# emtiyaz/vmp-for-svae

Hardware: AMD Instinct MI355X
Metric: vmp_step_datapoints_per_sec (higher is better)
Workload: dtype f32

## Files before the change

### vmp-for-svae_amd/csrc/vmp_mix.hip

```cpp
#include "vmp_common.h"
#include "vmp_linalg.h"
#include <stdlib.h>
#include <type_traits>

using namespace vmp;

namespace {

constexpr int TR = 64;
constexpr int LS = 68;
constexpr int MAX_NW = 8;
constexpr int MAX_NW1 = 8;
constexpr int max_nw(int KT) { return KT == 1 ? MAX_NW1 : MAX_NW; }
constexpr int MAX_BLOCKS = 1024;

struct PassArgs {
    const float* x;
    const float* r_in;
    const float* u_in;
    const uint8_t* mask;
    const float* pivot;
    const float* pack;
    float* r_out;
    float* u_out;
// ... 472 lines not shown
            } else {
                group(integral_constant<bool, false>{}, integral_constant<int, 0>{});
                group(integral_constant<bool, false>{}, integral_constant<int, 1>{});
                group(integral_constant<bool, false>{}, integral_constant<int, 2>{});
                group(integral_constant<bool, false>{}, integral_constant<int, 3>{});
            }

            if constexpr (STATS) {
                bf16x8 b[FT][3];
#pragma unroll
                for (int ft = 0; ft < FT; ++ft)
#pragma unroll
                    for (int t = 0; t < 3; ++t)
                        b[ft][t] = __builtin_bit_cast(bf16x8, u32x4{Bs[ft][t][0], Bs[ft][t][1], Bs[ft][t][2], Bs[ft][t][3]});
#pragma unroll
                for (int kt = 0; kt < KT; ++kt) {
                    bf16x8 av[3], rv[3];
#pragma unroll
                    for (int t = 0; t < 3; ++t) {
                        av[t] = __builtin_bit_cast(bf16x8, u32x4{As[kt][t][0], As[kt][t][1], As[kt][t][2], As[kt][t][3]});
                        if constexpr (SMM) rv[t] = __builtin_bit_cast(bf16x8, u32x4{Rs[kt][t][0], Rs[kt][t][1], Rs[kt][t][2], Rs[kt][t][3]});
                    }
#pragma unroll
                    for (int ta = 0; ta < MOM_TERMS; ++ta) {
#pragma unroll
                        for (int tb = 0; tb + ta < MOM_TERMS; ++tb) {
#pragma unroll
                            for (int ft = 0; ft < FT; ++ft) {
                                if (ta + tb == 0) acc[kt][ft] = __builtin_amdgcn_mfma_f32_16x16x32_bf16(av[ta], b[ft][tb], acc[kt][ft], 0, 0, 0);
                                else acs[kt][ft] = __builtin_amdgcn_mfma_f32_16x16x32_bf16(av[ta], b[ft][tb], acs[kt][ft], 0, 0, 0);
                            }
                        }
                        if constexpr (SMM) {
                            if (ta == 0) nacc[kt] = __builtin_amdgcn_mfma_f32_16x16x32_bf16(rv[ta], b[0][0], nacc[kt], 0, 0, 0);
                            else nacs[kt] = __builtin_amdgcn_mfma_f32_16x16x32_bf16(rv[ta], b[0][0], nacs[kt], 0, 0, 0);
                        }
                    }
                }
            }
        }

        if constexpr (STATS) {
            if (((row0 - lo) / TR) % VMP_MOM_FLUSH == VMP_MOM_FLUSH - 1 || row0 + TR >= hi) {
#pragma unroll
                for (int kt = 0; kt < KT; ++kt) {
#pragma unroll
                    for (int c = 0; c < 4; ++c) {
                        if constexpr (SMM) dn[kt][c] += (double)nacc[kt][c] + (double)nacs[kt][c];
#pragma unroll
                        for (int ft = 0; ft < FT; ++ft) dacc[kt][ft][c] += (double)acc[kt][ft][c] + (double)acs[kt][ft][c];
                    }
                    nacc[kt] = f32x4{0.f, 0.f, 0.f, 0.f};
                    nacs[kt] = f32x4{0.f, 0.f, 0.f, 0.f};
#pragma unroll
                    for (int ft = 0; ft < FT; ++ft) { acc[kt][ft] = f32x4{0.f, 0.f, 0.f, 0.f}; acs[kt][ft] = f32x4{0.f, 0.f, 0.f, 0.f}; }
                }
            }
        }
        __builtin_amdgcn_wave_barrier();
    }

    PASS_TS(2);
    if constexpr (STATS) pass_epilogue<D, KT, FLAV>(a, smem, dacc, dn, lane, wave, nw);
}


constexpr int AIS = 36;

struct FinArgs {
    const double* partials;
    const double* stats_in;
    int nblk, K, flavour, src, do_post;
    const float *alpha0, *beta0, *m0, *C0, *v0, *kappa;
    const float* pivot;
    float *alpha, *beta, *m, *C, *v, *xbar, *S, *pi, *pack;
    double* pack64;
    double* stats_out;
    double* peer[VMP_EXCH_MAX_RANKS];
    int nranks, rank;
    unsigned long long iter;
    int* status;
#ifdef VMP_DEBUG_TS
    long long* dbg_t;
#endif
};

#ifdef VMP_DEBUG_TS
#define FIN_TS(i) do { if (a.dbg_t && blockIdx.x == 0 && tid == 0) { a.dbg_t[i] = clock64(); if ((i) == 0) a.dbg_t[6] = wall_clock64(); if ((i) == 5) a.dbg_t[7] = wall_clock64(); } } while (0)
#else
#define FIN_TS(i) do { } while (0)
#endif
#ifdef VMP_DEBUG_TS
#define FIN_TSX(i, t) do { if (a.dbg_t && blockIdx.x == 0 && tid == (t)) a.dbg_t[i] = clock64(); } while (0)
#else
#define FIN_TSX(i, t) do { } while (0)
#endif

template <int D>
__device__ void finalize_block(const FinArgs& a, const int k, const int tid, const int nthreads);

template <int D> constexpr int xdl_wave_floats() { return Geo<D>::XROWS * LS + TR * AIS; }

template <int D, int FLAV, bool STATS, int MT = 3, bool GEN = true>
__device__ __forceinline__ void pass_xdl_body(const PassArgs& a) {
    using G = Geo<D>;
    constexpr int FT = G::FT, KT = 1;
    constexpr bool SMM = (FLAV == VMP_SMM);
    constexpr int DP = (D + 1) / 2;
    extern __shared__ __attribute__((aligned(16))) float smem[];
    const int lane = threadIdx.x & 63, wave = threadIdx.x >> 6, nw = blockDim.x >> 6;
    const int K = GEN ? a.K : 16;
    PASS_TS(0);
    float* xl = smem + wave * xdl_wave_floats<D>();
    unsigned* ai = reinterpret_cast<unsigned*>(xl + G::XROWS * LS);
    constexpr int ONE = D, ZERO = D + 1;
    const int ppos = (lane & ~15) + 4 * (lane & 3) + ((lane >> 2) & 3);

    const bool vec = a.vec_ok != 0;
    long long lo, hi;
    if (a.rpw_b == a.rpw) {
        lo = ((long long)blockIdx.x * nw + wave) * a.rpw;
        hi = lo + a.rpw;
    } else {
        const int hw = nw >> 1;
        const long long base = (long long)blockIdx.x * hw * (a.rpw + a.rpw_b);
        lo = wave < hw ? base + wave * a.rpw : base + hw * a.rpw + (wave - hw) * a.rpw_b;
        hi = lo + (wave < hw ? a.rpw : a.rpw_b);
    }
    if (hi > a.N) hi = a.N;
    float xr[D];
    {
        const long long n = lo + lane;
#pragma unroll
        for (int j = 0; j < D; ++j) xr[j] = 0.f;
        if (n < hi) load_row<D>(a.x + n * D, xr, vec);
    }
    const int i16 = lane & 15, kk = lane >> 4;
    float pv[D];
    {
        const float* __restrict__ pp = a.pivot ? a.pivot : a.x;
        const bool hasp = a.pivot != nullptr;
#pragma unroll
        for (int j = 0; j < D; ++j) { const float v = pp[j]; pv[j] = hasp ? v : 0.f; }
#pragma unroll
        for (int j = 0; j < D; ++j) pv[j] = __builtin_bit_cast(float, __builtin_amdgcn_readfirstlane(__builtin_bit_cast(int, pv[j])));
    }

    constexpr int NS = D < 4 ? D : 4;
    constexpr int NB = D > 4 ? D - 4 : 0;
    constexpr int QK = 3 * NS + 4 * NB, QS = QK | 1;
    static_assert(16 * QS * 4 <= xdl_wave_floats<D>(), "the operand image must fit the LDS of a one-wave launch");
    u32x4 Bsm[NS], B1[NB > 0 ? NB : 1], B2[NB > 0 ? NB : 1];
    v2f pch;
    float pua, pub;
    {
        const bool on = i16 < K;
        const float* __restrict__ pc = a.pack + (on ? i16 : 0) * G::PACK + D + G::TRI;
        const float c0 = pc[0], c1 = pc[1], c2 = pc[2], c3 = pc[3];
        pch.x = on ? c0 : -INFINITY;
        pch.y = on ? c1 : 0.f;
        pua = on ? c2 : 0.f;
        pub = on ? c3 : 1.f;
    }
    {
        u32x4* img = reinterpret_cast<u32x4*>(smem);
        for (int it = threadIdx.x; it < 16 * D; it += blockDim.x) {
            const int k = it / D, i = it - k * D;
            const bool on = k < K;
            const float* __restrict__ p = a.pack + (on ? k : 0) * G::PACK;
            const int tri = i * (i + 1) / 2;
            float mr[D], wr[D];
#pragma unroll
            for (int j = 0; j < D; ++j) { mr[j] = p[j]; wr[j] = p[D + tri + j]; }
            double bi = 0.0;
#pragma unroll
            for (int j = 0; j < D; ++j)
                if (j <= i) bi -= (double)wr[j] * ((double)mr[j] - (double)pv[j]);
            unsigned tb[3];
            split_bf16<3>(v2f{(float)bi, 0.f}, tb);
            const unsigned bias0 = (tb[0] & 0xffffu) | (tb[1] << 16), bias1 = tb[2] & 0xffffu;
            unsigned th[4] = {0u, 0u, 0u, 0u}, tm[4] = {0u, 0u, 0u, 0u}, tl[4] = {0u, 0u, 0u, 0u};
#pragma unroll
            for (int q = 0; q < DP; ++q) {
                const int j0 = 2 * q, j1 = 2 * q + 1;
                const float wa = j0 <= i ? wr[j0] : 0.f;
                const float wb = (j1 <= i && j1 < D) ? wr[j1 < D ? j1 : 0] : 0.f;
                unsigned t3[3];
                split_bf16<3>(v2f{wa, wb}, t3);
                th[q] = t3[0]; tm[q] = t3[1]; tl[q] = t3[2];
            }
            const u32x4 zero = u32x4{0u, 0u, 0u, 0u};
            const u32x4 bias = on ? u32x4{bias0, bias1, 0u, 0u} : zero;
            if (i < NS) {
                u32x4* o = img + k * QS + 3 * i;
                o[0] = on ? u32x4{th[0], th[1], tm[0], tm[1]} : zero;
                o[1] = on ? u32x4{th[0], th[1], tl[0], tl[1]} : zero;
                o[2] = bias;
            } else {
                u32x4* o = img + k * QS + 3 * NS + 4 * (i - 4);
                o[0] = on ? u32x4{th[0], th[1], th[2], th[3]} : zero;
                o[1] = on ? u32x4{tm[0], tm[1], tm[2], tm[3]} : zero;
                o[2] = on ? u32x4{tl[0], tl[1], tl[2], tl[3]} : zero;
                o[3] = bias;
            }
        }
        __syncthreads();
        const u32x4* q = img + i16 * QS;
        const int s0 = kk == 1 ? 1 : (kk == 3 ? 2 : 0);
#pragma unroll
        for (int i = 0; i < NS; ++i) Bsm[i] = q[3 * i + s0];
        if constexpr (NB > 0) {
            const int s1 = kk == 1 ? 3 : (kk == 2 ? 1 : 0), s2 = kk == 0 ? 2 : (kk == 1 ? 0 : 1);
#pragma unroll
            for (int ib = 0; ib < NB; ++ib) {
                B1[ib] = q[3 * NS + 4 * ib + s1];
                const u32x4 w2 = q[3 * NS + 4 * ib + s2];
                B2[ib] = kk == 3 ? u32x4{0u, 0u, 0u, 0u} : w2;
            }
        }
        __syncthreads();
    }
    xl[ONE * LS + lane] = 1.0f;
    xl[ZERO * LS + lane] = 0.0f;
    {
        u32x4 ones = u32x4{0x3F803F80u, 0x00003F80u, 0u, 0u}, zeros = u32x4{0u, 0u, 0u, 0u};
        *reinterpret_cast<u32x4*>(ai + lane * AIS + 12) = ones;
        *reinterpret_cast<u32x4*>(ai + lane * AIS + 16) = zeros;
    }
    const int rho = 4 * (i16 & 3) + (i16 >> 2);
    const int offA1 = rho * AIS + (kk == 1 ? 12 : (kk == 3 ? 4 : 0));
    const int offA2 = rho * AIS + (kk == 0 ? 0 : (kk == 1 ? 8 : (kk == 2 ? 4 : 16)));
    const int offA3 = rho * AIS + (kk == 3 ? 12 : 20 + 4 * kk);

    int offA[FT], offB[FT];
#pragma unroll
    for (int ft = 0; ft < FT; ++ft) {
        const int f = ft * 16 + i16;
        int ra = ZERO, rb = ZERO;
        if (f == 0) { ra = ONE; rb = ONE; }
        else if (f <= D) { ra = f - 1; rb = ONE; }
        else if (f < G::F) {
            int p = f - D - 1, d = 0;
            while (p >= D - d) { p -= D - d; ++d; }
            ra = d; rb = d + p;
        }
        offA[ft] = ra * LS + 4 * kk;
        offB[ft] = rb * LS + 4 * kk;
    }

    f32x4 acc[KT][FT], acs[KT][FT];
    double dacc[KT][FT][4];
    double dn[KT][4];
    float nsum = 0.f;
    double dnl = 0.0;
#pragma unroll
    for (int c = 0; c < 4; ++c) dn[0][c] = 0.0;
#pragma unroll
    for (int ft = 0; ft < FT; ++ft) {
        acc[0][ft] = f32x4{0.f, 0.f, 0.f, 0.f};
        acs[0][ft] = f32x4{0.f, 0.f, 0.f, 0.f};
#pragma unroll
        for (int c = 0; c < 4; ++c) dacc[0][ft][c] = 0.0;
    }

#ifdef VMP_DEBUG_TS
    asm volatile("" :: "v"(xr[0]), "v"(pv[0]), "v"(pch.x), "v"(Bsm[0][0]));
    asm volatile("s_waitcnt vmcnt(0)" ::: "memory");
#endif
    PASS_TS(1);
    long long row0 = lo, tbase = 0;
    int trows = TR;
    auto stage = [&](auto whole_c) __attribute__((always_inline)) {
        constexpr bool WHOLE = decltype(whole_c)::value;
        {
            const bool valid = WHOLE || row0 + lane < hi;
            float xs[2 * DP];
#pragma unroll
            for (int j = 0; j < 2 * DP; ++j) xs[j] = (valid && j < D) ? xr[j < D ? j : 0] - pv[j < D ? j : 0] : 0.f;
#pragma unroll
            for (int j = 0; j < D; ++j) xl[j * LS + ppos] = xs[j];
            unsigned th[4] = {0u, 0u, 0u, 0u}, tm[4] = {0u, 0u, 0u, 0u}, tl[4] = {0u, 0u, 0u, 0u};
#pragma unroll
            for (int q = 0; q < DP; ++q) {
                unsigned t3[3];
                split_bf16<3>(v2f{xs[2 * q], xs[2 * q + 1]}, t3);
                th[q] = t3[0]; tm[q] = t3[1]; tl[q] = t3[2];
            }
            *reinterpret_cast<u32x4*>(ai + lane * AIS) = u32x4{th[0], th[1], th[2], th[3]};
            *reinterpret_cast<u32x4*>(ai + lane * AIS + 4) = u32x4{tm[0], tm[1], tm[2], tm[3]};
            *reinterpret_cast<u32x4*>(ai + lane * AIS + 8) = u32x4{tl[0], tl[1], tl[2], tl[3]};
            *reinterpret_cast<u32x4*>(ai + lane * AIS + 20) = u32x4{th[0], th[1], th[0], th[1]};
            *reinterpret_cast<u32x4*>(ai + lane * AIS + 24) = u32x4{tm[0], tm[1], th[0], th[1]};
            *reinterpret_cast<u32x4*>(ai + lane * AIS + 28) = u32x4{tl[0], tl[1], tm[0], tm[1]};
            long long nb = row0 + TR;
            if (!GEN && WHOLE && nb < hi && nb > hi - TR) nb = hi - TR;
            const long long n2 = nb + lane;
#pragma unroll
            for (int j = 0; j < D; ++j) xr[j] = 0.f;
            if (n2 < hi) load_row<D>(a.x + n2 * D, xr, vec);
        }
        __builtin_amdgcn_wave_barrier();
        tbase = (row0 + kk) * (WHOLE ? 16 : K) + i16;
    };
    int othr = 0;
    auto body = [&](auto full_c, auto n0_v, auto ovl_c) __attribute__((always_inline)) {
        constexpr bool FULL = decltype(full_c)::value;
        constexpr bool LINE = !std::is_same<decltype(n0_v), int>::value;
        constexpr bool OVL = decltype(ovl_c)::value;
        static_assert(!OVL || LINE, "only a straight-line tile overlaps");
        const int n0 = n0_v;
        unsigned As[3][4], Bs[FT][3][4];
        auto subtile = [&](auto jj_c) __attribute__((always_inline)) {
            constexpr int jj = decltype(jj_c)::value;
            const int n16 = n0 + 16 * jj;
            if (!FULL && n16 >= trows) {
                if constexpr (STATS) {
#pragma unroll
                    for (int t = 0; t < 3; ++t) {
                        As[t][2 * jj] = 0u; As[t][2 * jj + 1] = 0u;
#pragma unroll
                        for (int ft = 0; ft < FT; ++ft) { Bs[ft][t][2 * jj] = 0u; Bs[ft][t][2 * jj + 1] = 0u; }
                    }
                }
                return;
            }
            f32x4 y[D];
            {
                const bf16x8 a3 = __builtin_bit_cast(bf16x8, *reinterpret_cast<const u32x4*>(ai + n16 * AIS + offA3));
#pragma unroll
                for (int i = 0; i < NS; ++i)
                    y[i] = __builtin_amdgcn_mfma_f32_16x16x32_bf16(a3, __builtin_bit_cast(bf16x8, Bsm[i]), f32x4{0.f, 0.f, 0.f, 0.f}, 0, 0, 0);
            }
            if constexpr (NB > 0) {
                const bf16x8 a1 = __builtin_bit_cast(bf16x8, *reinterpret_cast<const u32x4*>(ai + n16 * AIS + offA1));
                const bf16x8 a2 = __builtin_bit_cast(bf16x8, *reinterpret_cast<const u32x4*>(ai + n16 * AIS + offA2));
#pragma unroll
                for (int i = 0; i < NB; ++i)
                    y[4 + i] = __builtin_amdgcn_mfma_f32_16x16x32_bf16(a1, __builtin_bit_cast(bf16x8, B1[i]), f32x4{0.f, 0.f, 0.f, 0.f}, 0, 0, 0);
#pragma unroll
                for (int i = 0; i < NB; ++i)
                    y[4 + i] = __builtin_amdgcn_mfma_f32_16x16x32_bf16(a2, __builtin_bit_cast(bf16x8, B2[i]), y[4 + i], 0, 0, 0);
            }
            f32x4 q4 = y[0] * y[0], q4b = f32x4{0.f, 0.f, 0.f, 0.f};
#pragma unroll
            for (int i = 1; i < D; ++i) {
                if (i & 1) q4b = __builtin_elementwise_fma(y[i], y[i], q4b);
                else q4 = __builtin_elementwise_fma(y[i], y[i], q4);
            }
            q4 += q4b;
            v2f lg[2], uu[2], rr[2], w[2];
#pragma unroll
            for (int h = 0; h < 2; ++h) {
                const v2f qh = v2f{q4[2 * h], q4[2 * h + 1]};
                lg[h] = pk_const_minus_scaled(qh, pch);
                if constexpr (SMM) uu[h] = v2f{pua * __builtin_amdgcn_rcpf(qh.x + pub), pua * __builtin_amdgcn_rcpf(qh.y + pub)};
            }
            if constexpr (LINE) {
                static_assert(FULL, "straight-line tiles are whole tiles");
                const float mxs = row16_rs4_max(lg[0], lg[1]);
                lg[0] = v2f{__builtin_amdgcn_exp2f(lg[0].x - row16_bcast_bank<0>(mxs)), __builtin_amdgcn_exp2f(lg[0].y - row16_bcast_bank<1>(mxs))};
                lg[1] = v2f{__builtin_amdgcn_exp2f(lg[1].x - row16_bcast_bank<2>(mxs)), __builtin_amdgcn_exp2f(lg[1].y - row16_bcast_bank<3>(mxs))};
                const float invs = __builtin_amdgcn_rcpf(row16_rs4_sum(lg[0], lg[1]));
                rr[0] = v2f{lg[0].x * row16_bcast_bank<0>(invs), lg[0].y * row16_bcast_bank<1>(invs)};
                rr[1] = v2f{lg[1].x * row16_bcast_bank<2>(invs), lg[1].y * row16_bcast_bank<3>(invs)};
#pragma unroll
                for (int h = 0; h < 2; ++h) w[h] = SMM ? rr[h] * uu[h] : rr[h];
            } else {
                v2f mx[2], ssum[2];
#pragma unroll
                for (int h = 0; h < 2; ++h) {
                    mx[h] = row16_max2(lg[h]);
                    lg[h] = v2f{__builtin_amdgcn_exp2f(lg[h].x - mx[h].x), __builtin_amdgcn_exp2f(lg[h].y - mx[h].y)};
                    ssum[h] = row16_sum2(lg[h]);
                }
#pragma unroll
                for (int h = 0; h < 2; ++h) {
                    v2f inv = v2f{__builtin_amdgcn_rcpf(ssum[h].x), __builtin_amdgcn_rcpf(ssum[h].y)};
                    if constexpr (!FULL) {
                        const bool va = row0 + n16 + 8 * h + kk < hi, vb = row0 + n16 + 8 * h + 4 + kk < hi;
                        inv = v2f{va ? inv.x : 0.f, vb ? inv.y : 0.f};
                    }
                    rr[h] = lg[h] * inv;
                    w[h] = SMM ? rr[h] * uu[h] : rr[h];
                }
            }
#pragma unroll
            for (int v = 0; v < 4; ++v) {
                const float rv = rr[v >> 1][v & 1];
                if constexpr (FULL) {
                    float* __restrict__ ro = a.r_out + tbase + (long long)(n16 + 4 * v) * 16;
                    __builtin_nontemporal_store(rv, ro);
                    if constexpr (SMM) __builtin_nontemporal_store(uu[v >> 1][v & 1], a.u_out + tbase + (long long)(n16 + 4 * v) * 16);
                    if constexpr (!LINE)
                        if (a.logr_out) a.logr_out[tbase + (long long)(n16 + 4 * v) * 16] = logf(rv);
                } else {
                    const bool sv = (row0 + n16 + 4 * v + kk < hi) && i16 < K;
                    const long long o = tbase + (long long)(n16 + 4 * v) * K;
                    if (sv) {
                        a.r_out[o] = rv;
                        if constexpr (SMM) a.u_out[o] = uu[v >> 1][v & 1];
                        if (a.logr_out) a.logr_out[o] = logf(rv);
                    }
                }
            }
            if constexpr (LINE) {
                if (a.logr_out) {
#pragma unroll
                    for (int v = 0; v < 4; ++v) a.logr_out[tbase + (long long)(n16 + 4 * v) * 16] = logf(rr[v >> 1][v & 1]);
                }
            }
            if constexpr (STATS) {
                if constexpr (OVL) {
#pragma unroll
                    for (int h = 0; h < 2; ++h) {
                        const bool ka = n16 + 8 * h >= othr, kb = n16 + 8 * h + 4 >= othr;
                        w[h] = v2f{ka ? w[h].x : 0.f, kb ? w[h].y : 0.f};
                        if constexpr (SMM) rr[h] = v2f{ka ? rr[h].x : 0.f, kb ? rr[h].y : 0.f};
                    }
                }
                unsigned t3[3];
#pragma unroll
                for (int h = 0; h < 2; ++h) {
                    split_bf16<MT>(w[h], t3);
#pragma unroll
                    for (int t = 0; t < 3; ++t) As[t][2 * jj + h] = t3[t];
                }
                if constexpr (SMM) nsum += (rr[0].x + rr[0].y) + (rr[1].x + rr[1].y);
#pragma unroll
                for (int ft = 0; ft < FT; ++ft) {
                    const f32x4 fa = *reinterpret_cast<const f32x4*>(&xl[offA[ft] + n16]);
                    const f32x4 fb = *reinterpret_cast<const f32x4*>(&xl[offB[ft] + n16]);
                    const f32x4 pr = fa * fb;
#pragma unroll
                    for (int h = 0; h < 2; ++h) {
                        split_bf16<MT>(v2f{pr[2 * h], pr[2 * h + 1]}, t3);
#pragma unroll
                        for (int t = 0; t < 3; ++t) Bs[ft][t][2 * jj + h] = t3[t];
                    }
                }
            }
        };
        using std::integral_constant;
        subtile(integral_constant<int, 0>{});
        subtile(integral_constant<int, 1>{});

        if constexpr (STATS) {
            bf16x8 b[FT][3];
#pragma unroll
            for (int ft = 0; ft < FT; ++ft)
#pragma unroll
                for (int t = 0; t < 3; ++t)
                    b[ft][t] = __builtin_bit_cast(bf16x8, u32x4{Bs[ft][t][0], Bs[ft][t][1], Bs[ft][t][2], Bs[ft][t][3]});
            bf16x8 av[3];
#pragma unroll
            for (int t = 0; t < 3; ++t) av[t] = __builtin_bit_cast(bf16x8, u32x4{As[t][0], As[t][1], As[t][2], As[t][3]});
#pragma unroll
            for (int ta = 0; ta < MT; ++ta) {
#pragma unroll
                for (int tb = 0; tb + ta < MT; ++tb) {
#pragma unroll
                    for (int ft = 0; ft < FT; ++ft) {
                        if (ta + tb == 0) acc[0][ft] = __builtin_amdgcn_mfma_f32_16x16x32_bf16(av[ta], b[ft][tb], acc[0][ft], 0, 0, 0);
                        else acs[0][ft] = __builtin_amdgcn_mfma_f32_16x16x32_bf16(av[ta], b[ft][tb], acs[0][ft], 0, 0, 0);
                    }
                }
            }
        }
    };

    auto flush = [&]() __attribute__((always_inline)) {
        if constexpr (STATS) {
            if (((row0 - lo) / TR) % VMP_MOM_FLUSH == VMP_MOM_FLUSH - 1 || row0 + TR >= hi) {
#pragma unroll
                for (int c = 0; c < 4; ++c) {
#pragma unroll
                    for (int ft = 0; ft < FT; ++ft) dacc[0][ft][c] += (double)acc[0][ft][c] + (double)acs[0][ft][c];
                }
                if constexpr (SMM) { dnl += (double)nsum; nsum = 0.f; }
#pragma unroll
                for (int ft = 0; ft < FT; ++ft) { acc[0][ft] = f32x4{0.f, 0.f, 0.f, 0.f}; acs[0][ft] = f32x4{0.f, 0.f, 0.f, 0.f}; }
            }
        }
        __builtin_amdgcn_wave_barrier();
    };

    using std::integral_constant;
    using T_ = integral_constant<bool, true>;
    using F_ = integral_constant<bool, false>;
    if constexpr (!GEN) {
        for (; row0 + TR <= hi; row0 += TR) {
            stage(T_{});
            body(T_{}, integral_constant<int, 0>{}, F_{});
            body(T_{}, integral_constant<int, 32>{}, F_{});
            flush();
        }
        PASS_TS(6);
        if (row0 < hi && hi - lo >= TR) {
            const int done = TR - (int)(hi - row0);
            row0 = hi - TR;
            othr = done - kk;
            stage(T_{});
            if (done < 32) body(T_{}, integral_constant<int, 0>{}, T_{});
            body(T_{}, integral_constant<int, 32>{}, T_{});
            flush();
        }
    } else {
        if (K == 16) {
            for (; row0 + TR <= hi; row0 += TR) {
                stage(T_{});
                body(T_{}, integral_constant<int, 0>{}, F_{});
                body(T_{}, integral_constant<int, 32>{}, F_{});
                flush();
            }
        }
        PASS_TS(6);
        for (; row0 < hi; row0 += TR) {
            trows = (hi - row0 < TR) ? (int)(hi - row0) : TR;
            stage(F_{});
#pragma unroll 1
            for (int n0 = 0; n0 < trows; n0 += 32) {
                const bool full = (K == 16) && (n0 + 32 <= trows);
                if (full) body(T_{}, n0, F_{});
                else body(F_{}, n0, F_{});
            }
            flush();
        }
    }

    PASS_TS(2);
    if constexpr (STATS && SMM) {
        double tot = dnl;
        {
            int lo = __double2loint(tot), hi = __double2hiint(tot);
            tot += __hiloint2double(__shfl_xor(hi, 32), __shfl_xor(lo, 32));
            lo = __double2loint(tot); hi = __double2hiint(tot);
            tot += __hiloint2double(__shfl_xor(hi, 16), __shfl_xor(lo, 16));
        }
#pragma unroll
        for (int c = 0; c < 4; ++c) {
            const int src = 4 * kk + c;
            const int lo = __shfl(__double2loint(tot), src), hi = __shfl(__double2hiint(tot), src);
            dn[0][c] = __hiloint2double(hi, lo);
        }
    }
    if constexpr (STATS) pass_epilogue<D, 1, FLAV>(a, smem, dacc, dn, lane, wave, nw);
}

template <int D, int FLAV, bool STATS, int MT = 3>
__global__ __launch_bounds__(MAX_NW1 * WAVE) void pass_xdl_kernel(PassArgs a) {
    pass_xdl_body<D, FLAV, STATS, MT, true>(a);
}
template <int D, int FLAV, bool STATS, int MT = 3>
__global__ __launch_bounds__(MAX_NW1 * WAVE) void pass_xdl_overlap_kernel(PassArgs a) {
    pass_xdl_body<D, FLAV, STATS, MT, false>(a);
}

template <int D>
__device__ void write_pack(float* pack, int k, const double* m, const double* W ,
                           double c, double h, double ua, double ub) {
    using G = Geo<D>;
    float* p = pack + k * G::PACK;
    int idx = D;
    for (int j = 0; j < D; ++j) p[j] = (float)m[j];
    for (int i = 0; i < D; ++i)
        for (int j = 0; j <= i; ++j) p[idx++] = (float)W[i * D + j];
    const double LOG2E = 1.4426950408889634074;
    p[idx++] = (float)(c * LOG2E); p[idx++] = (float)(h * LOG2E); p[idx++] = (float)ua; p[idx++] = (float)ub;
}

__device__ __forceinline__ double fast_rsqrt_d(double x) {
    double y = __builtin_amdgcn_rsq(x);
    y = y * (1.5 - 0.5 * x * y * y);
    y = y * (1.5 - 0.5 * x * y * y);
    return y;
}

template <int D>
__device__ __forceinline__ void wave_chol_inverse(const double* A, int lane, double (&X)[D], double& sumlog, bool& ok) {
    double row[D], rd[D];
#pragma unroll
    for (int e = 0; e < D; ++e)
        row[e] = lane < D ? 0.5 * (A[lane * D + e] + A[e * D + lane]) : (e == lane ? 1.0 : 0.0);
    ok = true;
    double mydiag = 1.0;
#pragma unroll
    for (int j = 0; j < D; ++j) {
        double t = row[j];
#pragma unroll
        for (int p = 0; p < j; ++p) t -= row[p] * readlane_d(row[p], j);
        const double sj = readlane_d(t, j);
        ok = ok && (sj > 0.0);
        rd[j] = fast_rsqrt_d(sj);
        if (lane == j) mydiag = sj;
        row[j] = lane >= j ? t * rd[j] : 0.0;
    }
    double lg = lane < D ? 0.5 * log(mydiag) : 0.0;
    sumlog = 0.0;
#pragma unroll
    for (int j = 0; j < D; ++j) sumlog += readlane_d(lg, j);
#pragma unroll
    for (int i = 0; i < D; ++i) {
        double acc = (i == lane) ? 1.0 : 0.0;
#pragma unroll
        for (int p = 0; p < i; ++p) acc -= readlane_d(row[p], i) * X[p];
        X[i] = acc * rd[i];
    }
}

template <int D>
__device__ void estep_constants(int k, int flavour, double alpha_k, double alpha_sum, double beta_k, double v_k,
                                double logdetP, double kap, double& c, double& h, double& ua, double& ub, double& elp) {
    const double LOG2 = 0.69314718055994530942, PI = 3.14159265358979323846;
    elp = digamma_d(alpha_k) - digamma_d(alpha_sum);
    double sdg = 0.0;
    if (flavour == VMP_GMM) {
        for (int i = 0; i < D; ++i) sdg += digamma_d(0.5 * (v_k + 1.0 + i));
        const double ld = (logdetP > log(1e-20)) ? logdetP : 0.0;
        const double eld = sdg + D * LOG2 + ld;
        c = elp + 0.5 * eld - 0.5 * (D / beta_k);
        h = 0.5; ua = 1.0; ub = 1.0;
    } else {
        for (int i = 0; i < D; ++i) sdg += digamma_d(0.5 * (v_k + i));
        const double eld = sdg + D * LOG2 + logdetP;
        h = 0.5 * (D + kap);
        c = lgamma(0.5 * (D + kap)) - lgamma(0.5 * kap) - 0.5 * D * log(kap * PI) + elp + 0.5 * eld
            - h * (D / beta_k) + log(kap);
        ua = D + kap;
        ub = D / beta_k + kap;
    }
}

constexpr int FIN_THREADS = 1024;
constexpr int FIN_MAX_GROUPS = FIN_THREADS / 64;

__device__ __forceinline__ void st_pack(const FinArgs& a, int idx, double v) {
    a.pack[idx] = (float)v;
    if (a.pack64) a.pack64[idx] = v;
}

template <int D>
__device__ void finalize_block(const FinArgs& a, const int k, const int tid, const int nthreads) {
    using G = Geo<D>;
    __shared__ double part[FIN_MAX_GROUPS][64];
    __shared__ double st[G::SW];
    __shared__ double ntot;
    __shared__ double Ck[D * D], mk[D], sp[8], scal[8];
    __shared__ double alpha0s[VMP_MAX_K];
    const int K = a.K;
    const int FIN_GROUPS = nthreads >> 6;
    const bool post = a.do_post != 0;
    const bool smm = a.flavour == VMP_SMM;
    const double beta0 = post ? (double)a.beta0[k] : 0.0, v0 = post ? (double)a.v0[k] : 0.0;
    const double alpha0 = post ? (double)a.alpha0[k] : 0.0;
    const double kap = (post && smm) ? (double)a.kappa[k] : 0.0;
    bool shifted = (a.src == 0) && (a.pivot != nullptr);
    double m0d = 0.0, m0e = 0.0, C0de = 0.0, cd = 0.0, ce = 0.0;
    if (tid < D * D) {
        const int d = tid / D, e = tid % D;
        if (post) { m0d = a.m0[k * D + d]; m0e = a.m0[k * D + e]; C0de = a.C0[(k * D + d) * D + e]; }
        if (shifted) { cd = a.pivot[d]; ce = a.pivot[e]; }
    }
    if (post && tid < K) alpha0s[tid] = a.alpha0[tid];

    FIN_TS(0);
    if (a.src == 0) {
        constexpr int PX = G::PF + 1;
        const int f = tid & 63, g = tid >> 6;
        const double* __restrict__ mine = a.partials + (long long)k * MAX_BLOCKS * PX;
        int lo = 0, hi = f - (1 + D);
#pragma unroll
        for (int j = 0; j < D; ++j)
            if (lo == j && hi >= D - j) { hi -= D - j; lo = j + 1; }
        hi += lo;
        for (int lg = g; lg < FIN_MAX_GROUPS; lg += FIN_GROUPS) {
            double s = 0.0;
            for (int b0 = lg; b0 < a.nblk; b0 += FIN_MAX_GROUPS * 16) {
                double v1[16];
                const int fc = f < PX ? f : PX - 1;
#pragma unroll
                for (int i = 0; i < 16; ++i) {
                    const int b = b0 + i * FIN_MAX_GROUPS;
                    const int bc = b < a.nblk ? b : a.nblk - 1;
                    v1[i] = mine[(long long)bc * PX + fc];
                }
#pragma unroll
                for (int i = 0; i < 16; ++i) {
                    const bool in = b0 + i * FIN_MAX_GROUPS < a.nblk;
                    v1[i] = (in && f < PX) ? v1[i] : 0.0;
                }
#pragma unroll
                for (int i = 0; i < 16; ++i) s += v1[i];
            }
            part[lg][f] = s;
        }
        __syncthreads();
        FIN_TS(1);
        if (tid < 64) {
            double t1 = 0.0;
            for (int gg = 0; gg < FIN_MAX_GROUPS; ++gg) t1 += part[gg][tid];
            if (f == G::F) st[0] = t1;
            if (f == 0) st[1] = t1;
            if (f == G::PF) ntot = t1;
            if (f >= 1 && f < 1 + D) st[2 + (f - 1)] = t1;
            if (f >= 1 + D && f < G::F) { st[2 + D + lo * D + hi] = t1; st[2 + D + hi * D + lo] = t1; }
        }
    } else {
        for (int i = tid; i < G::SW; i += nthreads) st[i] = a.stats_in[(long long)k * G::SW + i];
        if (tid == 0) {
            double t = 0.0;
            for (int j = 0; j < K; ++j) t += a.stats_in[(long long)j * G::SW];
            ntot = t;
        }
    }
    __syncthreads();
    if (a.nranks >= 1) {
        constexpr int SWP = (G::SW + 1 + 7) & ~7;
        const int par = (int)(a.iter & 1), G_ = a.nranks;
        double val = 0.0;
        if (tid < G::SW) {
            val = st[tid];
            if (shifted && tid >= 2) {
                const double W = st[1];
                if (tid < 2 + D) {
                    val += W * (double)a.pivot[tid - 2];
                } else {
                    const int d = (tid - 2 - D) / D, e = (tid - 2 - D) % D;
                    const double pd = a.pivot[d], pe = a.pivot[e];
                    val += pd * st[2 + e] + st[2 + d] * pe + W * pd * pe;
                }
            }
        } else if (tid == G::SW) {
            val = ntot;
        }
        if (tid <= G::SW) {
            for (int g = 0; g < G_; ++g) {
                double* slot = a.peer[g] + (((size_t)par * G_ + a.rank) * K + k) * SWP;
                __hip_atomic_store(slot + tid, val, __ATOMIC_RELAXED, __HIP_MEMORY_SCOPE_SYSTEM);
            }
            __builtin_amdgcn_fence(__ATOMIC_RELEASE, "");
            asm volatile("s_waitcnt vmcnt(0)" ::: "memory");
        }
        __syncthreads();
        if (tid == 0) {
            __builtin_amdgcn_fence(__ATOMIC_RELEASE, "");
            asm volatile("s_waitcnt vmcnt(0)" ::: "memory");
            for (int g = 0; g < G_; ++g) {
                unsigned long long* fl = reinterpret_cast<unsigned long long*>(a.peer[g] + (size_t)2 * G_ * K * SWP);
                __hip_atomic_store(fl + ((size_t)par * G_ + a.rank) * K + k, a.iter + 1ull, __ATOMIC_RELAXED, __HIP_MEMORY_SCOPE_SYSTEM);
            }
        }
        double* mine = a.peer[a.rank];
        if (tid < G_) {
            const unsigned long long* fl = reinterpret_cast<const unsigned long long*>(mine + (size_t)2 * G_ * K * SWP)
                                           + ((size_t)par * G_ + tid) * K + k;
            const long long t0 = wall_clock64();
            bool ok = false;
            while (!ok) {
                ok = __hip_atomic_load(fl, __ATOMIC_RELAXED, __HIP_MEMORY_SCOPE_SYSTEM) == a.iter + 1ull;
                if (!ok) {
                    if (wall_clock64() - t0 > 400000000ll) break;
                    __builtin_amdgcn_s_sleep(8);
                }
            }
            if (!ok && a.status) *a.status = 1;
        }
        __syncthreads();
        if (tid == 0) __builtin_amdgcn_fence(__ATOMIC_ACQUIRE, "");
        __syncthreads();
        if (tid <= G::SW) {
            double s2 = 0.0;
            for (int g = 0; g < G_; ++g)
                s2 += __hip_atomic_load(mine + (((size_t)par * G_ + g) * K + k) * SWP + tid, __ATOMIC_RELAXED, __HIP_MEMORY_SCOPE_SYSTEM);
            if (tid < G::SW) st[tid] = s2; else ntot = s2;
        }
        shifted = false;
        cd = 0.0; ce = 0.0;
        __syncthreads();
    }
    if (a.stats_out) {
        for (int i = tid; i < G::SW; i += nthreads) {
            double val = st[i];
            if (shifted && i >= 2) {
                const double W = st[1];
                if (i < 2 + D) {
                    val += W * (double)a.pivot[i - 2];
                } else {
                    const int d = (i - 2 - D) / D, e = (i - 2 - D) % D;
                    const double pd = a.pivot[d], pe = a.pivot[e];
                    val += pd * st[2 + e] + st[2 + d] * pe + W * pd * pe;
                }
            }
            a.stats_out[(long long)k * G::SW + i] = val;
        }
    }
    if (!a.do_post) return;

    const double Nk = st[0], Wk = smm ? st[1] : st[0];
    const double* sx = st + 2;
    const double* sxx = st + 2 + D;
    const double den = smm ? (Wk + 1e-20) : Wk;
    const bool empty = (!smm) && !(Wk != 0.0);
    const double alpha_k = alpha0 + Nk;
    const double beta_k = beta0 + Wk;
    const double v_k = smm ? (v0 + Nk) : (v0 + Nk + 1.0);
    FIN_TS(2);
    if (tid < D * D) {
        const int d = tid / D, e = tid % D;
// ... 749 lines not shown
```

Measured before the change: 24.41 billion.

## Interleave MFMA energy computation with softmax post-processing across 16-row subtiles

Adds a specialised path for non-generic D=8, MT=2 stats passes that software-pipelines each 64-row tile. The MFMA energy products for the next 16-row subtile are issued while the softmax, stores and bf16 splitting of the current subtile run, with sched_barriers pinning the order. The aim is to hide MFMA latency behind VALU and transcendental work. It duplicates the body logic in a new code path, which raises register pressure and adds maintenance risk.

```diff
diff --git a/vmp-for-svae_amd/csrc/vmp_mix.hip b/vmp-for-svae_amd/csrc/vmp_mix.hip
--- a/vmp-for-svae_amd/csrc/vmp_mix.hip
+++ b/vmp-for-svae_amd/csrc/vmp_mix.hip
@@ -798,6 +798,7 @@
         __builtin_amdgcn_wave_barrier();
         tbase = (row0 + kk) * (WHOLE ? 16 : K) + i16;
     };
+    constexpr bool IL = !GEN && STATS && D == 8 && MT == 2;
     int othr = 0;
     auto body = [&](auto full_c, auto n0_v, auto ovl_c) __attribute__((always_inline)) {
         constexpr bool FULL = decltype(full_c)::value;
@@ -984,21 +985,189 @@
     using T_ = integral_constant<bool, true>;
     using F_ = integral_constant<bool, false>;
     if constexpr (!GEN) {
-        for (; row0 + TR <= hi; row0 += TR) {
-            stage(T_{});
-            body(T_{}, integral_constant<int, 0>{}, F_{});
-            body(T_{}, integral_constant<int, 32>{}, F_{});
-            flush();
-        }
-        PASS_TS(6);
-        if (row0 < hi && hi - lo >= TR) {
-            const int done = TR - (int)(hi - row0);
-            row0 = hi - TR;
-            othr = done - kk;
-            stage(T_{});
-            if (done < 32) body(T_{}, integral_constant<int, 0>{}, T_{});
-            body(T_{}, integral_constant<int, 32>{}, T_{});
-            flush();
+        if constexpr (IL) {
+            auto epart_a = [&](const int n16, f32x4 (&y)[D]) __attribute__((always_inline)) {
+                const bf16x8 a3 = __builtin_bit_cast(bf16x8, *reinterpret_cast<const u32x4*>(ai + n16 * AIS + offA3));
+#pragma unroll
+                for (int i = 0; i < NS; ++i)
+                    y[i] = __builtin_amdgcn_mfma_f32_16x16x32_bf16(a3, __builtin_bit_cast(bf16x8, Bsm[i]), f32x4{0.f, 0.f, 0.f, 0.f}, 0, 0, 0);
+            };
+            auto epart_b = [&](const int n16, f32x4 (&y)[D]) __attribute__((always_inline)) {
+                const bf16x8 a1 = __builtin_bit_cast(bf16x8, *reinterpret_cast<const u32x4*>(ai + n16 * AIS + offA1));
+                const bf16x8 a2 = __builtin_bit_cast(bf16x8, *reinterpret_cast<const u32x4*>(ai + n16 * AIS + offA2));
+#pragma unroll
+                for (int i = 0; i < NB; ++i)
+                    y[4 + i] = __builtin_amdgcn_mfma_f32_16x16x32_bf16(a1, __builtin_bit_cast(bf16x8, B1[i]), f32x4{0.f, 0.f, 0.f, 0.f}, 0, 0, 0);
+#pragma unroll
+                for (int i = 0; i < NB; ++i)
+                    y[4 + i] = __builtin_amdgcn_mfma_f32_16x16x32_bf16(a2, __builtin_bit_cast(bf16x8, B2[i]), y[4 + i], 0, 0, 0);
+            };
+            auto qform = [&](const f32x4 (&y)[D]) __attribute__((always_inline)) {
+                f32x4 q4 = y[0] * y[0], q4b = f32x4{0.f, 0.f, 0.f, 0.f};
+#pragma unroll
+                for (int i = 1; i < D; ++i) {
+                    if (i & 1) q4b = __builtin_elementwise_fma(y[i], y[i], q4b);
+                    else q4 = __builtin_elementwise_fma(y[i], y[i], q4);
+                }
+                q4 += q4b;
+                return q4;
+            };
+            auto post = [&](auto ovl_c, auto jj_c, const int n16, const f32x4 q4, unsigned (&As)[3][4], unsigned (&Bs)[FT][3][4],
+                            v2f (&rk)[2], auto mid) __attribute__((always_inline)) {
+                constexpr bool OVL = decltype(ovl_c)::value;
+                constexpr int jj = decltype(jj_c)::value;
+                v2f lg[2], uu[2], rr[2], w[2];
+#pragma unroll
+                for (int h = 0; h < 2; ++h) {
+                    const v2f qh = v2f{q4[2 * h], q4[2 * h + 1]};
+                    lg[h] = pk_const_minus_scaled(qh, pch);
+                    if constexpr (SMM) uu[h] = v2f{pua * __builtin_amdgcn_rcpf(qh.x + pub), pua * __builtin_amdgcn_rcpf(qh.y + pub)};
+                }
+                const float mxs = row16_rs4_max(lg[0], lg[1]);
+                lg[0] = v2f{__builtin_amdgcn_exp2f(lg[0].x - row16_bcast_bank<0>(mxs)), __builtin_amdgcn_exp2f(lg[0].y - row16_bcast_bank<1>(mxs))};
+                lg[1] = v2f{__builtin_amdgcn_exp2f(lg[1].x - row16_bcast_bank<2>(mxs)), __builtin_amdgcn_exp2f(lg[1].y - row16_bcast_bank<3>(mxs))};
+                const float invs = __builtin_amdgcn_rcpf(row16_rs4_sum(lg[0], lg[1]));
+                rr[0] = v2f{lg[0].x * row16_bcast_bank<0>(invs), lg[0].y * row16_bcast_bank<1>(invs)};
+                rr[1] = v2f{lg[1].x * row16_bcast_bank<2>(invs), lg[1].y * row16_bcast_bank<3>(invs)};
+#pragma unroll
+                for (int h = 0; h < 2; ++h) { w[h] = SMM ? rr[h] * uu[h] : rr[h]; rk[h] = rr[h]; }
+#pragma unroll
+                for (int v = 0; v < 4; ++v) {
+                    const long long o = tbase + (long long)(n16 + 4 * v) * 16;
+                    __builtin_nontemporal_store(rr[v >> 1][v & 1], a.r_out + o);
+                    if constexpr (SMM) __builtin_nontemporal_store(uu[v >> 1][v & 1], a.u_out + o);
+                }
+                mid();
+                if constexpr (OVL) {
+#pragma unroll
+                    for (int h = 0; h < 2; ++h) {
+                        const bool ka = n16 + 8 * h >= othr, kb = n16 + 8 * h + 4 >= othr;
+                        w[h] = v2f{ka ? w[h].x : 0.f, kb ? w[h].y : 0.f};
+                        if constexpr (SMM) rr[h] = v2f{ka ? rr[h].x : 0.f, kb ? rr[h].y : 0.f};
+                    }
+                }
+                if constexpr (SMM) {
+                    float s0 = rr[0].x + rr[0].y, s1 = rr[1].x + rr[1].y;
+                    asm volatile("" : "+v"(s0), "+v"(s1));
+                    nsum += s0 + s1;
+                }
+                unsigned t3[3];
+#pragma unroll
+                for (int h = 0; h < 2; ++h) {
+                    split_bf16<MT>(w[h], t3);
+#pragma unroll
+                    for (int t = 0; t < 3; ++t) As[t][2 * jj + h] = t3[t];
+                }
+#pragma unroll
+                for (int ft = 0; ft < FT; ++ft) {
+                    const f32x4 fa = *reinterpret_cast<const f32x4*>(&xl[offA[ft] + n16]);
+                    const f32x4 fb = *reinterpret_cast<const f32x4*>(&xl[offB[ft] + n16]);
+                    const f32x4 pr = fa * fb;
+#pragma unroll
+                    for (int h = 0; h < 2; ++h) {
+                        split_bf16<MT>(v2f{pr[2 * h], pr[2 * h + 1]}, t3);
+#pragma unroll
+                        for (int t = 0; t < 3; ++t) Bs[ft][t][2 * jj + h] = t3[t];
+                    }
+                }
+            };
+            auto moments = [&](const unsigned (&As)[3][4], const unsigned (&Bs)[FT][3][4]) __attribute__((always_inline)) {
+                bf16x8 b[FT][3], av[3];
+#pragma unroll
+                for (int t = 0; t < 3; ++t) {
+                    av[t] = __builtin_bit_cast(bf16x8, u32x4{As[t][0], As[t][1], As[t][2], As[t][3]});
+#pragma unroll
+                    for (int ft = 0; ft < FT; ++ft) b[ft][t] = __builtin_bit_cast(bf16x8, u32x4{Bs[ft][t][0], Bs[ft][t][1], Bs[ft][t][2], Bs[ft][t][3]});
+                }
+#pragma unroll
+                for (int ta = 0; ta < MT; ++ta) {
+#pragma unroll
+                    for (int tb = 0; tb + ta < MT; ++tb) {
+#pragma unroll
+                        for (int ft = 0; ft < FT; ++ft) {
+                            if (ta + tb == 0) acc[0][ft] = __builtin_amdgcn_mfma_f32_16x16x32_bf16(av[ta], b[ft][tb], acc[0][ft], 0, 0, 0);
+                            else acs[0][ft] = __builtin_amdgcn_mfma_f32_16x16x32_bf16(av[ta], b[ft][tb], acs[0][ft], 0, 0, 0);
+                        }
+                    }
+                }
+            };
+            auto tile = [&](auto half_c, auto ovl_c) __attribute__((always_inline)) {
+                using I0 = integral_constant<int, 0>;
+                using I1 = integral_constant<int, 1>;
+                constexpr bool HALF = decltype(half_c)::value;
+                f32x4 y[D], qa, qb;
+                unsigned As0[3][4], Bs0[FT][3][4], As1[3][4], Bs1[FT][3][4];
+                v2f rk[4][2];
+                auto none = [&]() __attribute__((always_inline)) { __builtin_amdgcn_sched_barrier(0); };
+                auto m16 = [&]() __attribute__((always_inline)) { __builtin_amdgcn_sched_barrier(0); epart_b(16, y); };
+                auto m32 = [&]() __attribute__((always_inline)) { __builtin_amdgcn_sched_barrier(0); epart_b(32, y); };
+                auto m48 = [&]() __attribute__((always_inline)) { __builtin_amdgcn_sched_barrier(0); epart_b(48, y); };
+                if constexpr (!HALF) {
+                    epart_a(0, y);
+                    epart_b(0, y);
+                    qa = qform(y);
+                    __builtin_amdgcn_sched_barrier(0);
+                    epart_a(16, y);
+                    post(ovl_c, I0{}, 0, qa, As0, Bs0, rk[0], m16);
+                    qb = qform(y);
+                    __builtin_amdgcn_sched_barrier(0);
+                    epart_a(32, y);
+                    post(ovl_c, I1{}, 16, qb, As0, Bs0, rk[1], m32);
+                    qa = qform(y);
+                    __builtin_amdgcn_sched_barrier(0);
+                    moments(As0, Bs0);
+                } else {
+                    epart_a(32, y);
+                    epart_b(32, y);
+                    qa = qform(y);
+                    __builtin_amdgcn_sched_barrier(0);
+                }
+                epart_a(48, y);
+                post(ovl_c, I0{}, 32, qa, As1, Bs1, rk[2], m48);
+                qb = qform(y);
+                __builtin_amdgcn_sched_barrier(0);
+                post(ovl_c, I1{}, 48, qb, As1, Bs1, rk[3], none);
+                __builtin_amdgcn_sched_barrier(0);
+                moments(As1, Bs1);
+                if (a.logr_out) {
+#pragma unroll
+                    for (int s = HALF ? 2 : 0; s < 4; ++s)
+#pragma unroll
+                        for (int v = 0; v < 4; ++v) a.logr_out[tbase + (long long)(16 * s + 4 * v) * 16] = logf(rk[s][v >> 1][v & 1]);
+                }
+            };
+            for (; row0 + TR <= hi; row0 += TR) {
+                stage(T_{});
+                tile(F_{}, F_{});
+                flush();
+            }
+            PASS_TS(6);
+            if (row0 < hi && hi - lo >= TR) {
+                const int done = TR - (int)(hi - row0);
+                row0 = hi - TR;
+                othr = done - kk;
+                stage(T_{});
+                if (done < 32) tile(F_{}, T_{});
+                else tile(T_{}, T_{});
+                flush();
+            }
+        } else {
+            for (; row0 + TR <= hi; row0 += TR) {
+                stage(T_{});
+                body(T_{}, integral_constant<int, 0>{}, F_{});
+                body(T_{}, integral_constant<int, 32>{}, F_{});
+                flush();
+            }
+            PASS_TS(6);
+            if (row0 < hi && hi - lo >= TR) {
+                const int done = TR - (int)(hi - row0);
+                row0 = hi - TR;
+                othr = done - kk;
+                stage(T_{});
+                if (done < 32) body(T_{}, integral_constant<int, 0>{}, T_{});
+                body(T_{}, integral_constant<int, 32>{}, T_{});
+                flush();
+            }
         }
     } else {
         if (K == 16) {
```

Result: faster. 25.13 billion (median of 6 runs) (+2.9%).
